# kepingbi/ProdSearch

Measured on AMD Instinct MI355X. Metric: train (u,q,i,neg) tuples/sec at bs=384, 20 neg, d=128, higher is better.
Workload: dtype f32 (fp32 MFMA and VALU; wide products, the fused per-replica kernels and grouped weight gradients as fp32-grade bf16x3 products: exact 3-way bf16 split of both fp32 operands, 6 of the 9 cross products as bf16 MFMAs per step, fp32 accumulation); 1 GPU; item_transformer d=128 1 layer 8 heads ff=512 uprev=20 bs=384/GPU 20 neg Q=8 W=1 P=18357 V=32387 dropout=0.10 (BASELINE configs[1]); global_batch=384, parallelism=dp1, step=sample+fwd+bwd+clip/Adam via nn.Module API (trainer.py:74-78), replicas_per_row=21

## Files before the change

include/prodsearch_hip.h:

```cpp
#ifndef PRODSEARCH_HIP_H
#define PRODSEARCH_HIP_H

#include <stddef.h>
#include <stdint.h>

#ifdef __cplusplus
extern "C" {
#endif

#define PS_MAX_LAYERS 8
#define PS_OK 0
#define PS_ERR_ARG 1
#define PS_ERR_HIP 2

typedef void* ps_stream_t;

enum { PS_MODEL_TEM = 0, PS_MODEL_QEM = 1,
       PS_MODEL_AEM = 2,
       PS_MODEL_ZAM = 3 };
enum { PS_QENC_FS = 0, PS_QENC_AVG = 1 };

typedef struct PsTemDesc {
  int32_t B;
  int32_t K;
// ... 48 lines not shown
  const int64_t *target_prod_idxs;
  const int64_t *u_item_idxs;
  const int64_t *pos_iword_idxs;
  const int64_t *neg_item_idxs;
  const int64_t *neg_word_idxs;
  const int64_t *candi_prod_idxs;
} PsTemBatch;

typedef struct PsTemWsLayout {
  int64_t total_floats;
  int32_t R;
  int32_t S;
  int64_t qmean, query_emb, x;
  int64_t kp, vp, qp, attn, ctx;
  int64_t y1, ln1, a1, h1, y2, enc;
  int64_t item_scores, word_scores, loss_parts;
  int64_t denc, dx;
} PsTemWsLayout;

const char* ps_version(void);
const char* ps_last_error(void);
const char* ps_arith_info(void);
int ps_set_fuse_bwd_min(int rows);
int ps_set_side_mode(int mode);
int ps_side_values_in_use(void);
void ps_side_abort(void);
void ps_debug_fail_fork(int nth);
int ps_set_deterministic(int on);
int ps_gemm_x3_config(int mode, int force_shape);
int ps_gemm_f32_weight(const float* A, int lda, const float* W, int tb, float* C, int ldc, int M, int N, int K,
                       const float* bias, float alpha, ps_stream_t stream);

int ps_tem_workspace_layout(const PsTemDesc* desc, PsTemWsLayout* out);

int ps_tem_forward(const PsTemDesc* desc, const PsTemTensors* params, const PsTemBatch* batch,
                   float* workspace, float* loss3, float* loss_acc, ps_stream_t stream);
int ps_tem_forward_sampled(const PsTemDesc* desc, const PsTemTensors* params, const PsTemBatch* batch,
                           const float* alias_prob, const int32_t* alias_idx, int64_t* neg_item_out, int64_t* neg_word_out,
                           float* workspace, float* loss3, float* loss_acc, ps_stream_t stream);

int ps_tem_backward(const PsTemDesc* desc, const PsTemTensors* params, const PsTemBatch* batch,
                    float* workspace, const PsTemTensors* grads, float loss_scale,
                    const float* loss_scale_dev ,
                    ps_stream_t stream);

int ps_gather_score(const PsTemDesc* desc, const PsTemTensors* params, const PsTemBatch* batch,
// ... 209 lines not shown
```

prodsearch_amd/_lib.py:

```python
import ctypes as C
import os

from . import build as _build

PS_MAX_LAYERS = 8
PS_MODEL_TEM, PS_MODEL_QEM, PS_MODEL_AEM, PS_MODEL_ZAM = 0, 1, 2, 3
PS_QENC_FS, PS_QENC_AVG = 0, 1

_f32p = C.POINTER(C.c_float)
_i64p = C.POINTER(C.c_int64)


class PsTemDesc(C.Structure):
    _fields_ = [(n, C.c_int32) for n in ('B', 'K', 'L', 'Q', 'W', 'C', 'd', 'H', 'F', 'n_layers')] + \
               [('product_size', C.c_int64), ('vocab_size', C.c_int64)] + \
               [(n, C.c_int32) for n in ('model', 'query_encoder', 'use_pos_emb', 'use_item_pos',
                                         'bias_product', 'pos_weight', 'sep_prod_emb', 'training')] + \
               [('dropout', C.c_float), ('seed', C.c_uint64), ('step', C.c_uint64)]


LAYER_FIELDS = ('wk', 'bk', 'wv', 'bv', 'wq', 'bq', 'wo', 'bo', 'w1', 'b1', 'w2', 'b2',
                'ff_ln_g', 'ff_ln_b', 'ln_g', 'ln_b')
TOP_FIELDS = ('product_emb', 'hist_product_emb', 'word_emb', 'product_bias', 'word_bias',
              'fs_w', 'fs_b', 'pe', 'final_ln_g', 'final_ln_b')
# ... 57 lines not shown


class PsRtmTensors(C.Structure):
    _fields_ = [(n, C.c_void_p) for n in RTM_TOP_FIELDS] + [('layer', PsLayerTensors * PS_MAX_LAYERS)]


class PsRtmBatch(C.Structure):
    _fields_ = [(n, C.c_void_p) for n in RTM_BATCH_FIELDS]


class PsRtmWsLayout(C.Structure):
    _fields_ = [('total_floats', C.c_int64)] + [(n, C.c_int32) for n in ('Bseq', 'S', 'J', 'pad_')] + \
               [(n, C.c_int64) for n in ('query_emb', 'valid', 'x', 'vec', 'cnt', 'enc', 'scores', 'weight',
                                         'pv_scores', 'dx')]


PS_RENC_PV, PS_RENC_PVC, PS_RENC_FS, PS_RENC_AVG = 0, 1, 2, 3

SYMBOLS = {
    'ps_version': (C.c_char_p, []),
    'ps_last_error': (C.c_char_p, []),
    'ps_arith_info': (C.c_char_p, []),
    'ps_set_fuse_bwd_min': (C.c_int, [C.c_int]),
    'ps_set_side_mode': (C.c_int, [C.c_int]),
    'ps_side_values_in_use': (C.c_int, []),
    'ps_set_deterministic': (C.c_int, [C.c_int]),
    'ps_side_abort': (None, []),
    'ps_debug_fail_fork': (None, [C.c_int]),
    'ps_gemm_x3_config': (C.c_int, [C.c_int, C.c_int]),
    'ps_gemm_f32_weight': (C.c_int, [C.c_void_p, C.c_int, C.c_void_p, C.c_int, C.c_void_p, C.c_int, C.c_int, C.c_int, C.c_int,
                                     C.c_void_p, C.c_float, C.c_void_p]),
    'ps_tem_workspace_layout': (C.c_int, [C.POINTER(PsTemDesc), C.POINTER(PsTemWsLayout)]),
    'ps_tem_forward': (C.c_int, [C.POINTER(PsTemDesc), C.POINTER(PsTemTensors), C.POINTER(PsTemBatch),
                                 C.c_void_p, C.c_void_p, C.c_void_p, C.c_void_p]),
    'ps_tem_forward_sampled': (C.c_int, [C.POINTER(PsTemDesc), C.POINTER(PsTemTensors), C.POINTER(PsTemBatch),
                                         C.c_void_p, C.c_void_p, C.c_void_p, C.c_void_p, C.c_void_p, C.c_void_p, C.c_void_p,
                                         C.c_void_p]),
    'ps_tem_backward': (C.c_int, [C.POINTER(PsTemDesc), C.POINTER(PsTemTensors), C.POINTER(PsTemBatch),
                                  C.c_void_p, C.POINTER(PsTemTensors), C.c_float, C.c_void_p, C.c_void_p]),
    'ps_gather_score': (C.c_int, [C.POINTER(PsTemDesc), C.POINTER(PsTemTensors), C.POINTER(PsTemBatch),
                                  C.c_void_p, C.c_void_p]),
    'ps_tem_score': (C.c_int, [C.POINTER(PsTemDesc), C.POINTER(PsTemTensors), C.POINTER(PsTemBatch),
                               C.c_void_p, C.c_void_p, C.c_void_p]),
    'ps_rtm_workspace_floats': (C.c_int, [C.POINTER(PsRtmDesc), C.c_int32, C.POINTER(C.c_int64)]),
    'ps_rtm_workspace_layout': (C.c_int, [C.POINTER(PsRtmDesc), C.c_int32, C.POINTER(PsRtmWsLayout)]),
    'ps_rtm_forward': (C.c_int, [C.POINTER(PsRtmDesc), C.POINTER(PsRtmTensors), C.POINTER(PsRtmBatch),
# ... 181 lines not shown
```

prodsearch_amd/csrc/mlp_fused.hip:

```cpp
#include "rowwise.h"
#include "x3frag.h"
#include <stdlib.h>
#ifndef TRY
#define TRY(x) do { int _rc = (x); if (_rc) return _rc; } while (0)
#endif

bool ps_fusion_enabled() {
  static const bool on = ps_env_int("PS_NO_FUSE", 0) == 0;
  return on;
}

#define MD 128
#define MBM 32
#define MT_THREADS 512
#define MLP_PF_DEFAULT 3
#define PLD 132

__device__ inline int opaque(int v) { asm volatile("" : "+v"(v)); return v; }

struct MlpTLds {
  uint16_t Xa[3][MBM * MD];
  float Ps[8][MBM * PLD];
  float vec[6][MD];
  float red[16];
// ... 366 lines not shown
  PS_REQUIRE(mlp_x3_enabled(a.F) && a.M > 0, "fused mlp: F=%d M=%d (F must be 256, 512 or 1024)", a.F, a.M);
  PS_REQUIRE(a.x3.on && a.x3.fwd_wo && a.x3.fwd_ff, "fused mlp: the weight fragment streams are missing (WSplit)");
  PS_REQUIRE(!a.fold_score || mlp_fwd_can_fold_score(a.M, a.F, MD), "fused mlp: folded scoring needs <= 65535 workgroups");
  KTimeScope kt("mlp_fwd", st);
  MlpFwdArgs as = a;
  as.stamp = g_mlp_stamp;
  const dim3 grid(ps_cdiv(a.M, MBM)), block(MT_THREADS);
  static bool a1 = false, a2 = false, a4 = false;
#ifdef PS_DIAG
  static bool ad1 = false, ad2 = false, ad3 = false;
  static const int diag = ps_diag_int("PS_MLP_DIAG", 0);
  if (a.F == 512 && diag == 1) { TRY(set_lds_attr(mlp_fwd_t_kernel<2, 3, 1>, ad1)); PS_KLAUNCH((mlp_fwd_t_kernel<2, 3, 1>), grid, block, sizeof(MlpTLds), st, as); }
  else if (a.F == 512 && diag == 2) { TRY(set_lds_attr(mlp_fwd_t_kernel<2, 3, 2>, ad2)); PS_KLAUNCH((mlp_fwd_t_kernel<2, 3, 2>), grid, block, sizeof(MlpTLds), st, as); }
  else if (a.F == 512 && diag == 3) { TRY(set_lds_attr(mlp_fwd_t_kernel<2, 3, 3>, ad3)); PS_KLAUNCH((mlp_fwd_t_kernel<2, 3, 3>), grid, block, sizeof(MlpTLds), st, as); }
  else
#endif
  if (a.F == 256) { TRY(set_lds_attr(mlp_fwd_t_kernel<1, 3>, a1)); PS_KLAUNCH((mlp_fwd_t_kernel<1, 3>), grid, block, sizeof(MlpTLds), st, as); }
  else if (a.F == 512) { TRY(set_lds_attr(mlp_fwd_t_kernel<2, 3>, a2)); PS_KLAUNCH((mlp_fwd_t_kernel<2, 3>), grid, block, sizeof(MlpTLds), st, as); }
  else { TRY(set_lds_attr(mlp_fwd_t_kernel<4, 3>, a4)); PS_KLAUNCH((mlp_fwd_t_kernel<4, 3>), grid, block, sizeof(MlpTLds), st, as); }
  PS_LAUNCH_CHECK();
  return PS_OK;
}

template <int NBW, int PF>
__global__ __launch_bounds__(MT_THREADS, 2) void mlp_bwd_t_kernel(const MlpBwdArgs a) {
  fork_signal(a.sig, a.sigval);
  extern __shared__ float lds_raw[];
  MlpTLds& L = *reinterpret_cast<MlpTLds*>(lds_raw);
  const int tid = threadIdx.x, lane = tid & 63, wave = __builtin_amdgcn_readfirstlane(tid >> 6), l31 = lane & 31, h = lane >> 5;
  const int m0 = blockIdx.x * MBM, M = a.M, F = a.F;
  const int mrow = 4 * wave + (lane >> 4), c8 = 8 * (lane & 15);
  const int mg = m0 + mrow;
  const bool ok = mg < M;
  const uint32_t step_ctx = drop_step(a.drop_ctx), step_ff1 = drop_step(a.drop_ff1), step_ff2 = drop_step(a.drop_ff2);
  MLP_STAMP(0);
  float (*Csum)[MBM][MD] = reinterpret_cast<float (*)[MBM][MD]>(&L.Ps[2][0]);
  static_assert(3 * MBM * MD <= 3 * MBM * PLD, "column-sum scratch must fit three partial slots");

  const uint16_t* ff_stream = a.x3.bwd_ff + (size_t)(wave * NBW) * 16 * 1536;
  uint4 ring[PF][3];
#pragma unroll
  for (int s = 0; s < PF; ++s) load_frag(ring[s], ff_stream, s, lane);
  if (tid < 64) {
    const int which = tid >> 5, q = tid & 31;
    *reinterpret_cast<float4*>(&L.vec[which][4 * q]) = *reinterpret_cast<const float4*>((which == 0 ? a.gf : a.g1) + 4 * q);
  }
  float x2[8], st2[2] = {0.f, 0.f};
  {
    const float* src = a.y2 + (size_t)(ok ? mg : 0) * MD + c8;
    const float4 v0 = ok ? *reinterpret_cast<const float4*>(src) : make_float4(0.f, 0.f, 0.f, 0.f);
    const float4 v1 = ok ? *reinterpret_cast<const float4*>(src + 4) : make_float4(0.f, 0.f, 0.f, 0.f);
    x2[0] = v0.x; x2[1] = v0.y; x2[2] = v0.z; x2[3] = v0.w; x2[4] = v1.x; x2[5] = v1.y; x2[6] = v1.z; x2[7] = v1.w;
    if (ok) { const float2 s2 = *reinterpret_cast<const float2*>(a.stf + 2 * (size_t)mg); st2[0] = s2.x; st2[1] = s2.y; }
  }
  float dy[8];
  if (a.item_scores) {
    const float invB = a.scale * (a.scale_dev ? *a.scale_dev : 1.f) / (float)a.B;
    const float wpos = a.pos_weight ? (float)a.K : 1.f;
    const int K1 = a.K + 1;
    const int mm = ok ? mg : 0;
    const int b = mm / K1, j = mm - b * K1;
    int64_t idx = j == 0 ? a.target[b] : a.neg_items[(size_t)b * a.K + j - 1];
    idx = idx < 0 ? a.P : (idx > a.P ? a.P : idx);
    const float sc = a.item_scores[mm];
    const float ds = ok ? (j == 0 ? wpos * (sigmoid_f(sc) - 1.f) : sigmoid_f(sc)) * invB : 0.f;
    const float* row = a.product_emb + (size_t)idx * MD + c8;
    const float4 v0 = *reinterpret_cast<const float4*>(row), v1 = *reinterpret_cast<const float4*>(row + 4);
    dy[0] = ds * v0.x; dy[1] = ds * v0.y; dy[2] = ds * v0.z; dy[3] = ds * v0.w;
    dy[4] = ds * v1.x; dy[5] = ds * v1.y; dy[6] = ds * v1.z; dy[7] = ds * v1.w;
  } else {
    const float* src = a.denc + (size_t)(ok ? mg : 0) * MD + c8;
    const float4 v0 = ok ? *reinterpret_cast<const float4*>(src) : make_float4(0.f, 0.f, 0.f, 0.f);
    const float4 v1 = ok ? *reinterpret_cast<const float4*>(src + 4) : make_float4(0.f, 0.f, 0.f, 0.f);
    dy[0] = v0.x; dy[1] = v0.y; dy[2] = v0.z; dy[3] = v0.w; dy[4] = v1.x; dy[5] = v1.y; dy[6] = v1.z; dy[7] = v1.w;
  }
  __syncthreads();
  MLP_STAMP(1);

  auto ln_bwd_stage = [&](const float (&dyv)[8], const float (&x)[8], const float mean, const float rstd, const int vg,
                          const bool has_res, const float (&res)[8], const DropSpec& drop, const uint32_t dstep,
                          float (&dxr)[8], float* out_dx, float* out_drop) {
    const float4 g0 = *reinterpret_cast<const float4*>(&L.vec[vg][c8]), g1 = *reinterpret_cast<const float4*>(&L.vec[vg][c8 + 4]);
    const float gg[8] = {g0.x, g0.y, g0.z, g0.w, g1.x, g1.y, g1.z, g1.w};
    float xh[8], dh[8], s1 = 0.f, s2 = 0.f;
#pragma unroll
    for (int j = 0; j < 8; ++j) {
      xh[j] = (x[j] - mean) * rstd;
      dh[j] = dyv[j] * gg[j];
      s1 += dh[j]; s2 += dh[j] * xh[j];
    }
    s1 = row16_sum(s1) * (1.f / MD);
    s2 = row16_sum(s2) * (1.f / MD);
// ... 54 lines not shown
  park(a.part_f);
  __syncthreads();
  MLP_STAMP(3);

  f32x16 acc2[4];
#pragma unroll
  for (int nb = 0; nb < 4; ++nb)
#pragma unroll
    for (int r = 0; r < 16; ++r) acc2[nb][r] = 0.f;
  const int mrow_p = m0 + l31;
  const bool row_ok = mrow_p < M;
  constexpr int NS = 16 * NBW;
#pragma unroll
  for (int bi = 0; bi < NBW; ++bi) {
    const int fb = wave * NBW + bi, f0 = 32 * fb + 16 * h;
    float* tile = &L.Ps[wave][0];
    float4 a1g[4];
    tile_load(a1g, a.a1 + (size_t)m0 * F + 32 * fb, F, lane, M - m0);
    f32x16 acc1;
#pragma unroll
    for (int r = 0; r < 16; ++r) acc1[r] = 0.f;
    uint4 bq[2][3];
    read_b(bq[0], L.Xa, l31, 8 * h);
    { if ((wave >= 4) == (bi == 0)) __builtin_amdgcn_s_setprio(2); else __builtin_amdgcn_s_setprio(1); }
#pragma unroll
    for (int t = 0; t < 8; ++t) {
      const int s = 16 * bi + t;
      if (t + 1 < 8) read_b(bq[(t + 1) & 1], L.Xa, l31, 16 * (t + 1) + 8 * h);
      __builtin_amdgcn_sched_barrier(0);
      x3_mma(acc1, ring[s % PF], bq[t & 1]);
      load_frag(ring[s % PF], ff_stream, s + PF < NS ? s + PF : NS - 1, lane);
      __builtin_amdgcn_sched_barrier(0);
    }
    { if ((wave >= 4) == (bi == 0)) __builtin_amdgcn_s_setprio(1); else __builtin_amdgcn_s_setprio(0); }
    MLP_STAMP(4 + 2 * bi);
    Philox4 r0 = {0u, 0u, 0u, 0u}, r1 = {0u, 0u, 0u, 0u};
    if (a.drop_ff1.thr) {
      r0 = drop_call16(a.drop_ff1, (uint32_t)mrow_p, (uint32_t)(f0 >> 3), step_ff1);
      r1 = drop_call16(a.drop_ff1, (uint32_t)mrow_p, (uint32_t)(f0 >> 3) + 1u, step_ff1);
    }
    float a1v[16];
    tile_load_put(tile, a1g, lane);
    tile_get(tile, a1v, l31, h);
    float dv[16];
#pragma unroll
    for (int r = 0; r < 16; ++r) {
// ... 1 lines not shown
      if (a.drop_ff1.thr) g *= drop_half(a.drop_ff1, r < 8 ? r0 : r1, r & 7);
      dv[r] = row_ok ? g : 0.f;
    }
    tile_put(tile + MBM * TLD, dv, l31, h);
    tile_store(tile + MBM * TLD, a.da1 + (size_t)m0 * F + 32 * fb, F, lane, M - m0);
    {
      float cs[16];
#pragma unroll
      for (int r = 0; r < 16; ++r) cs[r] = half_sum_last(dv[r]);
      if (l31 == 31) {
        float* pb = a.part_b1 + ((size_t)blockIdx.x * 3) * F + f0;
#pragma unroll
        for (int q = 0; q < 4; ++q) *reinterpret_cast<float4*>(pb + 4 * q) = make_float4(cs[4 * q], cs[4 * q + 1], cs[4 * q + 2], cs[4 * q + 3]);
      }
    }
    MLP_STAMP(5 + 2 * bi);
    { if ((wave >= 4) == (bi == 0)) __builtin_amdgcn_s_setprio(2); else __builtin_amdgcn_s_setprio(1); }
    uint4 df[2][3];
    {
      const float lo8[8] = {dv[0], dv[1], dv[2], dv[3], dv[4], dv[5], dv[6], dv[7]};
      const float hi8[8] = {dv[8], dv[9], dv[10], dv[11], dv[12], dv[13], dv[14], dv[15]};
      split8(lo8, df[0]);
      split8(hi8, df[1]);
    }
#pragma unroll
    for (int u = 0; u < 8; ++u) {
      const int s = 16 * bi + 8 + u;
      x3_mma(acc2[u & 3], ring[s % PF], df[u >> 2]);
      load_frag(ring[s % PF], ff_stream, s + PF < NS ? s + PF : NS - 1, lane);
      __builtin_amdgcn_sched_barrier(0);
    }
  }
  __builtin_amdgcn_s_setprio(0);
  MLP_STAMP(8);
  float x1[8], st1v[2] = {0.f, 0.f};
  {
    const float* src = a.y1 + (size_t)(ok ? mg : 0) * MD + c8;
    const float4 v0 = ok ? *reinterpret_cast<const float4*>(src) : make_float4(0.f, 0.f, 0.f, 0.f);
    const float4 v1 = ok ? *reinterpret_cast<const float4*>(src + 4) : make_float4(0.f, 0.f, 0.f, 0.f);
    x1[0] = v0.x; x1[1] = v0.y; x1[2] = v0.z; x1[3] = v0.w; x1[4] = v1.x; x1[5] = v1.y; x1[6] = v1.z; x1[7] = v1.w;
    if (ok) { const float2 s2 = *reinterpret_cast<const float2*>(a.st1 + 2 * (size_t)mg); st1v[0] = s2.x; st1v[1] = s2.y; }
  }
  const int kbo = wave & 3, nh = wave >> 2;
  const uint16_t* wo_stream = a.x3.bwd_wo + (size_t)(kbo * 8 + 4 * nh) * 1536;
  uint4 wof[4][3];
#pragma unroll
// ... 32 lines not shown
    dump_acc(L.Ps[nh], acc, l31, h, kbo);
  }
  __syncthreads();
  MLP_STAMP(12);
  if (ok) {
    const float* p0 = &L.Ps[0][mrow * PLD + c8];
    const float* p1 = &L.Ps[1][mrow * PLD + c8];
    const float4 u0 = *reinterpret_cast<const float4*>(p0), u1 = *reinterpret_cast<const float4*>(p0 + 4);
    const float4 w0 = *reinterpret_cast<const float4*>(p1), w1 = *reinterpret_cast<const float4*>(p1 + 4);
    float* q = a.dctx + (size_t)mg * MD + c8;
    *reinterpret_cast<float4*>(q) = make_float4(u0.x + w0.x, u0.y + w0.y, u0.z + w0.z, u0.w + w0.w);
    *reinterpret_cast<float4*>(q + 4) = make_float4(u1.x + w1.x, u1.y + w1.y, u1.z + w1.z, u1.w + w1.w);
  }
  MLP_STAMP(13);
}

int mlp_bwd_fused_blocks(int M) { return ps_cdiv(M, MBM); }
int mlp_bwd_b1_rows(int M, int F) { (void)F; return ps_cdiv(M, MBM); }

int launch_mlp_bwd_fused(const MlpBwdArgs& a, hipStream_t st) {
  PS_REQUIRE(mlp_x3_enabled(a.F) && a.M > 0, "fused mlp backward: F=%d M=%d (F must be 256, 512 or 1024)", a.F, a.M);
  PS_REQUIRE(a.part_f && a.part_1 && a.part_b1, "fused mlp backward: column sums must be parked");
  PS_REQUIRE(a.x3.on && a.x3.bwd_wo && a.x3.bwd_ff, "fused mlp backward: the weight fragment streams are missing (WSplit)");
  KTimeScope kt("mlp_bwd", st);
  MlpBwdArgs b = a;
  b.sig = nullptr; b.sigval = 0;
  b.stamp = g_mlp_stamp ? g_mlp_stamp + 128 : nullptr;
  const dim3 grid(ps_cdiv(a.M, MBM)), block(MT_THREADS);
  static bool a1 = false, a2 = false, a4 = false;
  if (a.F == 256) TRY(set_lds_attr(mlp_bwd_t_kernel<1, 3>, a1));
  else if (a.F == 512) TRY(set_lds_attr(mlp_bwd_t_kernel<2, 3>, a2));
  else TRY(set_lds_attr(mlp_bwd_t_kernel<4, 3>, a4));
  side_take_signal(st, &b.sig, &b.sigval);
  if (a.F == 256) hipLaunchKernelGGL((mlp_bwd_t_kernel<1, 3>), grid, block, sizeof(MlpTLds), st, b);
  else if (a.F == 512) hipLaunchKernelGGL((mlp_bwd_t_kernel<2, 3>), grid, block, sizeof(MlpTLds), st, b);
  else hipLaunchKernelGGL((mlp_bwd_t_kernel<4, 3>), grid, block, sizeof(MlpTLds), st, b);
  PS_LAUNCH_CHECK();
  return PS_OK;
}
```

prodsearch_amd/csrc/rowwise.h:

```cpp
#pragma once
#include "common.h"

struct ScoreArgs {
  int B, K, W, C, R, d;
  FDiv fK1, fWK1, fC;
  int64_t P, V;
  int bias_product, pos_weight;
  const int64_t* target; const int64_t* neg_items; const int64_t* pos_words; const int64_t* neg_words;
  const int64_t* candi;
  const float* product_emb; const float* word_emb; const float* product_bias; const float* word_bias;
  const float* enc;
  float* item_scores;
  float* word_scores;
  float* loss_parts;
  float* item_terms;
  float* word_terms;
  float* loss3;
  float* loss_acc;
  float* loss_blk;
  int loss_nblk;
  float scale;
  const float* scale_dev;
  float* denc;
  int part;
  float* g_product_emb; float* g_word_emb; float* g_product_bias; float* g_word_bias;
  float* word_blk; int word_nblk; float* item_blk; uint32_t* ticket;
  const float* samp_prob; const int32_t* samp_alias; uint32_t samp_step, samp_k0, samp_k1; int samp_inline;
  unsigned long long* stamp;
};
#define PS_WORD_TASKS_PER_WG 16
inline void score_finish(ScoreArgs& a) {
  a.fK1 = make_fdiv(a.K + 1); a.fWK1 = make_fdiv(a.W * (a.K + 1)); a.fC = make_fdiv(a.C > 0 ? a.C : 1);
}
int launch_score_fwd(ScoreArgs& a, hipStream_t st);
int launch_loss(const ScoreArgs& a, hipStream_t st);
int launch_score_bwd(const ScoreArgs& a, hipStream_t st);

struct WSplit {
  const float* w[3]; int rows[3], cols[3];
  uint16_t* fwd_wo; uint16_t* fwd_ff; uint16_t* bwd_ff; uint16_t* bwd_wo;
  int on;
  const float* wkv[2]; uint16_t* fwd_kv;
  uint16_t* bwd_kv;
};
__host__ __device__ inline int wsplit_chunks(const WSplit& W, int ) {
  const int d = W.cols[0], F = W.rows[1];
  return (d * d + 2 * d * F) / 8 + (W.wkv[0] ? 2 * d * d / 8 : 0);
// ... 205 lines not shown
struct MlpFwdArgs {
  int M, F;
  int fan, S, qpos;
  const float* ctx; const float* xin;
  const float *wo, *bo, *g1, *be1, *w1, *b1, *w2, *b2, *gf, *bef;
  DropSpec drop_ctx, drop_ff1, drop_ff2;
  float *y1, *ln1, *st1, *a1, *h1, *y2, *stf, *enc;
  int fold_score; ScoreArgs sc;
  WSplit x3;
  unsigned long long* stamp;
};
int launch_mlp_fwd_fused(const MlpFwdArgs& a, hipStream_t st);
bool mlp_fwd_can_fold_score(int M, int F, int d);
bool mlp_x3_enabled(int F);
bool mlp_fused_serves(int d, int F);
int64_t mlp_x3_floats(int d, int F);
bool ps_fusion_enabled();

struct MlpBwdArgs {
  int M, F;
  const float* denc;
  const float* item_scores; const int64_t* target; const int64_t* neg_items; const float* product_emb;
  int B, K, pos_weight; int64_t P; float scale; const float* scale_dev;
  const float* y2; const float* stf; const float* gf;
  const float* y1; const float* st1; const float* g1;
  const float* a1;
  const float *wo, *w1, *w2;
  DropSpec drop_ctx, drop_ff1, drop_ff2;
  float* do2;
  float* da1;
  float* dy1;
  float* dout;
  float* dctx;
  float* part_f;
  float* part_1;
  float* part_b1;
  WSplit x3;
  uint32_t* sig; uint32_t sigval;
  unsigned long long* stamp;
};
int launch_mlp_bwd_fused(const MlpBwdArgs& a, hipStream_t st);
int mlp_bwd_fused_blocks(int M);
int mlp_bwd_b1_rows(int M, int F);
```

prodsearch_amd/csrc/rowwise.hip:

```cpp
#include "rowwise.h"
#include <stdlib.h>

static inline int lpr_for(int d) {
  int n = d / 4, l = 1;
  while (l < n && l < 64) l <<= 1;
  return l;
}

__device__ inline int64_t clamp_idx(int64_t i, int64_t hi) { return i < 0 ? hi : (i > hi ? hi : i); }

struct Task {
  const float* row; const float* vec; float bias; float* out;
  float* term; float tw;
  float lw;
};
__device__ inline Task score_task(const ScoreArgs& a, int t) {
  Task k;
  const int K1 = a.K + 1;
  if (a.C > 0) {
    int b = fdiv(t, a.fC);
    int64_t idx = clamp_idx(a.candi[t], a.P);
    k.row = a.product_emb + (size_t)idx * a.d;
    k.vec = a.enc + (size_t)b * a.R * a.d;
    k.bias = a.bias_product ? a.product_bias[idx] : 0.f;
// ... 1438 lines not shown
      it.bias = 0.f;
    });
  det_owner_walk<EPL, WG>(a.B * a.W * K1, owner, nown, hl, d, a.g_word_emb, a.g_word_bias, a.V - 1, keys_word,
    [&](int u, DetItem& it) {
      const int b = fdiv(u, a.fWK1), r = u - b * a.W * K1, w = r / K1, j = r - w * K1;
      it.row = keys_word[u];
      const float s = a.word_scores[((size_t)b * a.W + w) * K1 + j];
      const float* prow = a.product_emb + (size_t)clamp_idx(a.target[b], a.P) * d;
      float pv[EPL];
#pragma unroll
      for (int k = 0; k < EPL; ++k) pv[k] = (WG && k < epl) ? prow[c + 32 * k] : 0.f;
      int cnt = 0;
      for (int w2 = 0; w2 < a.W; ++w2) cnt += (a.pos_words[(size_t)b * a.W + w2] != a.V - 1);
      const float ds = (j == 0 ? sigmoid_f(s) - 1.f : sigmoid_f(s)) * (invB / (float)(cnt > 0 ? cnt : 1));
#pragma unroll
      for (int k = 0; k < EPL; ++k) it.v[k] = ds * pv[k];
      it.bias = ds;
    });
}

int launch_score_bwd(const ScoreArgs& a, hipStream_t st) {
  PS_REQUIRE(a.d % 32 == 0 && a.d <= 32 * BW_MAXE, "score bwd: d=%d unsupported", a.d);
  if (ps_deterministic()) {
    if (a.denc && a.part != 2) {
      ScoreArgs e = a;
      e.part = 1;
      const int iw = a.R > 1 ? ps_cdiv(a.B * (a.K + 1), SB_RG) : 0;
      launch_score_bwd_kernel(e, (a.R > 1 ? 2 : 1) * a.B + iw, st);
      PS_LAUNCH_CHECK();
    }
    if (a.part != 1) {
      const size_t nkeys = (size_t)a.B * (a.K + 1) * (1 + a.W) + a.B;
      float* term = ps_det_scratch(1, (size_t)a.B * a.d + nkeys + 4, st);
      PS_REQUIRE(term, "score bwd: deterministic mode has no scratch (allocation failed or stream capture)");
      int32_t* keys = reinterpret_cast<int32_t*>(term + (size_t)a.B * a.d);
      hipLaunchKernelGGL(score_bwd_det_pre_kernel, dim3(ps_cdiv(a.B, 8)), dim3(256), 0, st, a, term, keys);
      PS_LAUNCH_CHECK();
      if (a.g_word_emb) {
        if (a.d <= 128) hipLaunchKernelGGL(score_bwd_det_kernel<4>, dim3(256), dim3(32 * SBD_OWNERS_PER_WG), 0, st, a, term, keys);
        else if (a.d <= 256) hipLaunchKernelGGL(score_bwd_det_kernel<8>, dim3(256), dim3(32 * SBD_OWNERS_PER_WG), 0, st, a, term, keys);
        else hipLaunchKernelGGL(score_bwd_det_kernel<16>, dim3(256), dim3(32 * SBD_OWNERS_PER_WG), 0, st, a, term, keys);
      } else {
        if (a.d <= 128) hipLaunchKernelGGL((score_bwd_det_kernel<4, false>), dim3(256), dim3(32 * SBD_OWNERS_PER_WG), 0, st, a, term, keys);
        else if (a.d <= 256) hipLaunchKernelGGL((score_bwd_det_kernel<8, false>), dim3(256), dim3(32 * SBD_OWNERS_PER_WG), 0, st, a, term, keys);
        else hipLaunchKernelGGL((score_bwd_det_kernel<16, false>), dim3(256), dim3(32 * SBD_OWNERS_PER_WG), 0, st, a, term, keys);
      }
      PS_LAUNCH_CHECK();
    }
    return PS_OK;
  }
  const int item_wgs = a.R > 1 ? ps_cdiv(a.B * (a.K + 1), SB_RG) : 0;
#if PS_DIAG_ON
  ScoreArgs as = a;
  as.stamp = ps_diag_int("PS_SBW_STAMP", 0) ? ps_debug_stamp_ptr() : nullptr;
  launch_score_bwd_kernel(as, (a.R > 1 ? 2 : 1) * a.B + item_wgs, st);
#else
  launch_score_bwd_kernel(a, (a.R > 1 ? 2 : 1) * a.B + item_wgs, st);
#endif
  PS_LAUNCH_CHECK();
  return PS_OK;
}

template <int EPL>
__device__ __forceinline__ void row_fetch_add(float* dst, const float* src, int c, float scale) {
  float v[EPL];
#pragma unroll
  for (int k = 0; k < EPL; ++k) v[k] = src[c + 32 * k];
#pragma unroll
  for (int k = 0; k < EPL; ++k) atomicAdd(&dst[c + 32 * k], scale == 1.f ? v[k] : v[k] * scale);
}
template <int EPL>
__device__ __forceinline__ void row_fetch_add2(float* dst, const float* src, const float* src2, int c) {
  float v[EPL], u[EPL];
#pragma unroll
// ... 455 lines not shown
```

prodsearch_amd/csrc/tem.hip:

```cpp
#include "encoder.h"
#include "graph.h"
#include <math.h>
#include <stdarg.h>
#include <stdio.h>
#include <string.h>

static thread_local char g_err[512] = "";
void ps_set_error(const char* fmt, ...) {
  va_list ap;
  va_start(ap, fmt);
  vsnprintf(g_err, sizeof(g_err), fmt, ap);
  va_end(ap);
}
extern "C" const char* ps_last_error(void) { return g_err; }
extern "C" const char* ps_version(void) { return "prodsearch_hip 0.1 (gfx950, fp32 MFMA)"; }
bool gemm_x3_on();
extern "C" const char* ps_arith_info(void) {
  return gemm_x3_on() ? "f32 (fp32 MFMA and VALU; wide products, the fused per-replica kernels and grouped weight gradients as fp32-grade "
                        "bf16x3 products: exact 3-way bf16 split of both fp32 operands, 6 of the 9 cross products as bf16 MFMAs per step, "
                        "fp32 accumulation)"
                      : "f32 (fp32 MFMA and VALU)";
}

#include <vector>
// ... 969 lines not shown
  PS_CHECK_HIP(hipMemcpyAsync(enc_out, workspace + w.enc, sizeof(float) * (size_t)D.B * D.d, hipMemcpyDeviceToDevice, st));
  return PS_OK;
}

static void park_colsums(LnBwdArgs& a, float* ws, const Ws& w, ColFoldList* fold) {
  if (!fold || fold->n >= PS_MAX_COLFOLD) return;
  ColFold& f = fold->e[fold->n];
  a.partial = ws + w.lnpart + (size_t)fold->n * w.lnrows * 3 * a.d;
  f.partial = a.partial; f.nblk = ln_bwd_blocks(a.rows); f.d = a.d;
  f.dst[0] = a.dgamma; f.dst[1] = a.dbeta; f.dst[2] = a.colsum;
  ++fold->n;
}

static int& fuse_bwd_min_slot() {
  static int v = ps_env_int("PS_FUSE_BWD_MIN", 1024);
  return v;
}
extern "C" int ps_set_fuse_bwd_min(int rows) {
  const int old = fuse_bwd_min_slot();
  fuse_bwd_min_slot() = rows;
  return old;
}

static thread_local GemmProblem g_wg3_last[4];
static thread_local int g_wg3_last_n = 0;
static thread_local bool g_wg3_defer_ok = false;
static int flush_wg3_last(hipStream_t st) {
  const int n = g_wg3_last_n;
  g_wg3_last_n = 0;
  return n ? run_wgrads(g_wg3_last, n, st) : PS_OK;
}
int enc_layers_backward(const PsTemDesc& D, const PsTemTensors& P, const PsTemTensors& G, const int64_t* ui,
                        const float* valid, float* ws, const Ws& w, hipStream_t st, ColFoldList* fold,
                        const ScoreArgs* score_on_side, bool rows_listed) {
  const bool drop = D.training && D.dropout > 0.f;
  const int B = D.B, d = D.d, S = w.S, NL = D.n_layers, F = D.F;
  PS_REQUIRE(G.final_ln_g && G.final_ln_b, "backward: null final LayerNorm gradient");
  LnBwdArgs f;
  memset(&f, 0, sizeof(f));
  f.dy = ws + w.denc; f.lddy = d; f.stats = ws + w.fin_stats; f.g = P.final_ln_g; f.d = d;
  f.dgamma = G.final_ln_g; f.dbeta = G.final_ln_b;
  side_set_light((int64_t)B * S * d <= ((int64_t)2 << 20));
  static const bool bwd_fuse_on = ps_env_int("PS_NO_FUSE_BWD", 0) == 0;
  const int bwd_fuse_min = fuse_bwd_min_slot();
  const bool fuse_last = NL > 0 && fold && bwd_fuse_on && ps_fusion_enabled() && w.layer[NL - 1].Sq == 1 &&
                         mlp_fused_serves(d, F) && w.wsplit && w.layer[NL - 1].M2 == w.Mf && w.Mf >= bwd_fuse_min &&
                         mlp_bwd_fused_blocks(w.Mf) <= w.lnrows && fold->n + 3 <= PS_MAX_COLFOLD;
  if (score_on_side && !(fuse_last && w.R > 1)) {
    ScoreArgs t = *score_on_side;
    t.denc = ws + w.denc;
    SideCtx* sc = side_ctx_on(st);
    if (sc && w.R > 1) {
      t.part = 1;
      TRY(launch_score_bwd(t, st));
      TRY(side_fork(st));
      t.part = 2;
      TRY(launch_score_bwd(t, sc->stream));
    } else {
      TRY(launch_score_bwd(t, st));
    }
    score_on_side = nullptr;
  }
  if (fuse_last) {
  } else if (NL > 0) {
    const LayerWs& l = w.layer[NL - 1];
    f.x = ws + l.y2; f.ldx = d; f.rows = w.Mf; f.dx = ws + w.dy2; f.lddx = d;
    f.colsum = G.layer[NL - 1].b2;
// ... 12 lines not shown
    const PsLayerTensors& Lp = P.layer[i];
    const PsLayerTensors& Lg = G.layer[i];
    PS_REQUIRE(Lg.wk && Lg.wv && Lg.wq && Lg.wo && Lg.w1 && Lg.w2 && Lg.bk && Lg.bv && Lg.bq && Lg.bo && Lg.b1 &&
               Lg.b2 && Lg.ff_ln_g && Lg.ff_ln_b, "backward: layer %d has null gradients", i);
    const float* xin = i == 0 ? ws + w.x : ws + w.layer[i - 1].y2;
    const float* xn = ws + l.xn;
    const int ns = l.n_in * S, M2 = l.M2;
    const float* do2 = drop ? ws + w.do2 : ws + w.dy2;
    const bool fused = fuse_last && i == NL - 1;
    static const bool wgrad_early = ps_diag_int("PS_WGRAD_LATE", 0) == 0;
    if (fused) {
      MlpBwdArgs m;
      memset(&m, 0, sizeof(m));
      m.M = M2; m.F = F;
      m.denc = ws + w.denc; m.y2 = ws + l.y2; m.stf = ws + w.fin_stats; m.gf = P.final_ln_g;
      m.y1 = ws + l.y1; m.st1 = ws + l.ff_stats; m.g1 = Lp.ff_ln_g; m.a1 = ws + l.a1;
      m.wo = Lp.wo; m.w1 = Lp.w1; m.w2 = Lp.w2;
      m.drop_ctx = make_drop(D, PS_SITE_CTX(i)); m.drop_ff1 = make_drop(D, PS_SITE_FF1(i));
      m.drop_ff2 = make_drop(D, PS_SITE_FF2(i));
      if (score_on_side) {
        const ScoreArgs& sa = *score_on_side;
        m.item_scores = sa.item_scores; m.target = sa.target; m.neg_items = sa.neg_items; m.product_emb = sa.product_emb;
        m.B = sa.B; m.K = sa.K; m.pos_weight = sa.pos_weight; m.P = sa.P; m.scale = sa.scale; m.scale_dev = sa.scale_dev;
      }
      m.x3 = make_wsplit(D, P, ws, w);
      m.do2 = const_cast<float*>(do2); m.da1 = ws + w.da1; m.dy1 = ws + w.dy1;
      m.dout = drop ? ws + w.do_ : ws + w.dy1; m.dctx = ws + w.dctx;
      const int nwg = mlp_bwd_fused_blocks(M2);
      {
        ColFold& c0 = fold->e[fold->n];
        m.part_f = ws + w.lnpart + (size_t)fold->n * w.lnrows * 3 * d;
        c0.partial = m.part_f; c0.nblk = nwg; c0.d = d;
        c0.dst[0] = G.final_ln_g; c0.dst[1] = G.final_ln_b; c0.dst[2] = Lg.b2;
        ++fold->n;
        ColFold& c1 = fold->e[fold->n];
        m.part_1 = ws + w.lnpart + (size_t)fold->n * w.lnrows * 3 * d;
        c1.partial = m.part_1; c1.nblk = nwg; c1.d = d;
        c1.dst[0] = Lg.ff_ln_g; c1.dst[1] = Lg.ff_ln_b; c1.dst[2] = Lg.bo;
        ++fold->n;
        ColFold& c2 = fold->e[fold->n];
        m.part_b1 = ws + w.gcpart;
        c2.partial = m.part_b1; c2.nblk = mlp_bwd_b1_rows(M2, F); c2.d = F;
        c2.dst[0] = Lg.b1; c2.dst[1] = nullptr; c2.dst[2] = nullptr;
        ++fold->n;
      }
      TRY(launch_mlp_bwd_fused(m, st));
      GemmProblem wg[1] = {gp_wgrad(do2, d, ws + l.h1, F, Lg.w2, d, F, M2)};
      GemmProblem wg1[1] = {gp_wgrad(ws + w.da1, F, ws + l.ln1, d, Lg.w1, F, d, M2)};
      GemmProblem wgo[1] = {gp_wgrad(m.dout, d, ws + l.ctx, d, Lg.wo, d, d, M2)};
      TRY(side_fork(st));
      if (score_on_side) {
        ScoreArgs t = *score_on_side;
        t.denc = nullptr;
        SideCtx* sc = side_ctx_on(st);
        TRY(launch_score_bwd(t, sc ? sc->stream : st));
      }
      static const int wg_group_rows = ps_diag_int("PS_WGRAD_GROUP_ROWS", (1 << 30));
      if (M2 <= wg_group_rows) {
        GemmProblem all3[3] = {wg[0], wg1[0], wgo[0]};
        TRY(side_run(all3, 3, st));
      } else {
        TRY(side_run(wg, 1, st));
        TRY(side_run(wg1, 1, st));
        TRY(side_run(wgo, 1, st));
      }
    } else {
      GemmProblem p = gp(do2, d, 0, Lp.w2, F, 1, ws + w.da1, F, M2, F, d);
      p.act = ACT_GELU_BWD; p.act_aux = ws + l.a1; p.drop = make_drop(D, PS_SITE_FF1(i)); p.colsum = Lg.b1;
      if (fold && fold->n < PS_MAX_COLFOLD && i == NL - 1) {
        ColFold& cf = fold->e[fold->n++];
        p.colsum_part = ws + w.gcpart;
        cf.partial = p.colsum_part; cf.nblk = 4 * ps_cdiv(M2, 64); cf.d = F;
        cf.dst[0] = Lg.b1; cf.dst[1] = nullptr; cf.dst[2] = nullptr;
      }
// ... 143 lines not shown
      if (drop) { n.out2 = ws + w.do2; n.drop2 = make_drop(D, PS_SITE_FF2(i - 1)); }
      n.colsum = G.layer[i - 1].b2; n.dgamma = Lg.ln_g; n.dbeta = Lg.ln_b;
      park_colsums(n, ws, w, fold);
      TRY(launch_ln_bwd(n, st));
    }
  }
  return PS_OK;
}

static int tem_backward_impl(const PsTemDesc* desc, const PsTemTensors* params, const PsTemBatch* batch,
                             float* ws, const PsTemTensors* grads, float loss_scale, const float* loss_scale_dev,
                             ps_stream_t stream);
extern "C" int ps_tem_backward(const PsTemDesc* desc, const PsTemTensors* params, const PsTemBatch* batch,
                               float* ws, const PsTemTensors* grads, float loss_scale, const float* loss_scale_dev,
                               ps_stream_t stream) {
  const int rc = tem_backward_impl(desc, params, batch, ws, grads, loss_scale, loss_scale_dev, stream);
  if (rc != PS_OK) { side_abort(); enc_clear_call_flags(); }
  return rc;
}
static int tem_backward_impl(const PsTemDesc* desc, const PsTemTensors* params, const PsTemBatch* batch,
                             float* ws, const PsTemTensors* grads, float loss_scale, const float* loss_scale_dev,
                             ps_stream_t stream) {
  enc_clear_call_flags();
  PS_REQUIRE(desc && params && batch && ws && grads, "backward: null argument");
  PsTemDesc D = *desc;
  D.C = 0;
  Ws w;
  TRY(make_ws(D, w));
  hipStream_t st = (hipStream_t)stream;
  const PsTemTensors& P = *params;
  const PsTemTensors& G = *grads;
  const bool tem = D.model == PS_MODEL_TEM;
  const bool drop = D.training && D.dropout > 0.f;
  const int B = D.B, d = D.d, S = w.S, NL = tem ? D.n_layers : 0, F = D.F;
  const float* hist = D.sep_prod_emb ? P.hist_product_emb : P.product_emb;
  float* ghist = D.sep_prod_emb ? G.hist_product_emb : G.product_emb;
  const bool word_grad = G.word_emb != nullptr;
  PS_REQUIRE(G.product_emb && G.word_bias && ghist && hist, "backward: null table gradient");
  PS_REQUIRE(!D.bias_product || G.product_bias, "backward: null product_bias gradient");

  ScoreArgs s;
  fill_score(D, P, *batch, ws, w, s);
  s.scale = loss_scale; s.scale_dev = loss_scale_dev; s.denc = ws + w.denc;
  s.g_product_emb = G.product_emb; s.g_word_emb = G.word_emb; s.g_product_bias = G.product_bias;
  s.g_word_bias = G.word_bias;
  static const bool score_side_on = ps_diag_int("PS_SCORE_BWD_MAIN", 0) == 0;
  const bool score_deferred = tem && NL > 0 && w.R > 1 && score_side_on;
  if (!score_deferred) TRY(launch_score_bwd(s, st));

  const float* wp_w[PS_WPLANES_MAX]; int wp_r[PS_WPLANES_MAX], wp_c[PS_WPLANES_MAX];
  const int wp_n = wplane_list(D, P, w, wp_w, wp_r, wp_c);
  WPlaneScope wplanes(st, wp_w, wp_r, wp_c, wp_n);
  ColFoldList fold;
  fold.n = 0;
  const float* dqe = ws + w.denc;
  int lddqe = d;
  if (tem) {
    g_wg3_defer_ok = true; g_wg3_last_n = 0;
    const int rc_enc = enc_layers_backward(D, P, G, batch->u_item_idxs, nullptr, ws, w, st, &fold, score_deferred ? &s : nullptr,
                                           rows_list_ok(D));
    g_wg3_defer_ok = false;
    if (rc_enc != PS_OK) { g_wg3_last_n = 0; return rc_enc; }
    dqe = ws + w.dx;
    lddqe = S * d;
  } else if (ps_model_attn(D.model)) {
    TRY(ae_backward(D, P, G, batch->u_item_idxs, ws, w, st));
    dqe = ws + w.ae_dqe;
  }

  bool fw_by_gemm = false;
  EmbedBwdArgs e;
  memset(&e, 0, sizeof(e));
  e.B = B; e.Q = D.Q; e.L = D.L; e.S = S; e.d = d; e.P = D.product_size; e.V = D.vocab_size; e.tem = tem;
  e.qw = batch->query_word_idxs; e.ui = batch->u_item_idxs; e.dx = ws + w.dx;
  if (enc_take_dx_two_partials()) e.dx2 = ws + w.dxn;
  e.drop_fs = make_drop(D, PS_SITE_FS);
  e.g_hist_tab = ghist; e.g_word_emb = G.word_emb;
  if (D.query_encoder == PS_QENC_FS) {
    PS_REQUIRE(G.fs_w && G.fs_b, "backward: null FS encoder gradient");
    e.fw_x = ws + w.qmean; e.g_fs_w = G.fs_w;
    if (ps_fusion_enabled() && d <= 128) {
      e.fsb_dqe = dqe; e.fsb_lddqe = lddqe; e.fsb_qe = ws + w.query_emb; e.fsb_w = P.fs_w; e.g_fs_b = G.fs_b;
      if (word_grad) e.det_dm = ws + w.dqmean;
      static const bool fw_gemm_on = ps_env_int("PS_FW_BY_GEMM", 1) != 0;
// ... 1 lines not shown
    } else {
      TRY(launch_tanh_bwd(dqe, lddqe, ws + w.query_emb, ws + w.dqpre, G.fs_b, B, d, st));
      if (word_grad) {
        GemmProblem p = gp(ws + w.dqpre, d, 0, P.fs_w, d, 1, ws + w.dqmean, d, B, d, d);
        p.no_deep = 1;
        TRY(run1(p, st));
        e.dqmean_d = ws + w.dqmean;
      }
      e.fw_dy = ws + w.dqpre;
    }
  } else if (word_grad) {
    PS_CHECK_HIP(hipMemcpy2DAsync(ws + w.dqmean, sizeof(float) * d, dqe, sizeof(float) * lddqe, sizeof(float) * d, B,
                                  hipMemcpyDeviceToDevice, st));
    e.dqmean_d = ws + w.dqmean;
  }
  e.fold = fold;
  const int rc_sc = launch_embed_scatter(e, st);
  if (rc_sc != PS_OK) { g_wg3_last_n = 0; return rc_sc; }
  if (fw_by_gemm) {
    PS_REQUIRE(g_wg3_last_n <= 3, "backward: deferred weight-gradient group is full");
    g_wg3_last[g_wg3_last_n++] = gp_wgrad(ws + w.dqpre, d, ws + w.qmean, d, G.fs_w, d, d, B);
  }
  TRY(flush_wg3_last(st));
  TRY(side_join(st));
  return PS_OK;
}

struct StageLayout { uint32_t* step_word; int64_t* p[6]; int n[6]; };
static StageLayout stage_layout(const PsTemDesc& D, float* ws, const Ws& w) {
  StageLayout L;
  L.step_word = reinterpret_cast<uint32_t*>(ws + w.stage);
  int64_t* base = reinterpret_cast<int64_t*>(ws + w.stage + 4);
  const int n[6] = {D.B * D.Q, D.B * D.L, D.B, D.B * D.W, D.B * D.K, D.B * D.W * D.K};
  int64_t off = 0;
  for (int k = 0; k < 6; ++k) { L.p[k] = base + off; L.n[k] = n[k]; off += (n[k] + 1) & ~1; }
  return L;
}
static PsTemBatch staged_batch(const StageLayout& L) {
  PsTemBatch b;
  memset(&b, 0, sizeof(b));
  b.query_word_idxs = L.p[0]; b.u_item_idxs = L.p[1]; b.target_prod_idxs = L.p[2]; b.pos_iword_idxs = L.p[3];
  b.neg_item_idxs = L.p[4]; b.neg_word_idxs = L.p[5];
  return b;
}

extern "C" int ps_graph_replay_enabled(void) { return ps_graphs_enabled() ? 1 : 0; }
// ... 182 lines not shown
```

Before: 35.22 million tuples/s.

## Fuse item-embedding gradient scatter into the fused MLP backward kernel

Adds a templated ISC path to the fused MLP backward kernel. Each wave reads the score gradient and item index per row and atomically adds ds*enc into the product-embedding and bias gradients, interleaved with the MFMA loop. The separate score backward on the side stream then skips the item rows and only handles word gradients, launched after the deferred weight-gradient flush. This removes a separate item-scatter pass and its reread of enc. In exchange it adds atomics and registers inside a hot kernel and moves the word scatter later, onto the main stream.

```diff
diff --git a/include/prodsearch_hip.h b/include/prodsearch_hip.h
--- a/include/prodsearch_hip.h
+++ b/include/prodsearch_hip.h
@@ -94,6 +94,8 @@
 const char* ps_last_error(void);
 const char* ps_arith_info(void);
 int ps_set_fuse_bwd_min(int rows);
+int ps_set_item_scatter_fused(int on);
+int ps_item_scatter_fused_taken(void);
 int ps_set_side_mode(int mode);
 int ps_side_values_in_use(void);
 void ps_side_abort(void);
diff --git a/prodsearch_amd/_lib.py b/prodsearch_amd/_lib.py
--- a/prodsearch_amd/_lib.py
+++ b/prodsearch_amd/_lib.py
@@ -103,6 +103,8 @@
     'ps_last_error': (C.c_char_p, []),
     'ps_arith_info': (C.c_char_p, []),
     'ps_set_fuse_bwd_min': (C.c_int, [C.c_int]),
+    'ps_set_item_scatter_fused': (C.c_int, [C.c_int]),
+    'ps_item_scatter_fused_taken': (C.c_int, []),
     'ps_set_side_mode': (C.c_int, [C.c_int]),
     'ps_side_values_in_use': (C.c_int, []),
     'ps_set_deterministic': (C.c_int, [C.c_int]),
diff --git a/prodsearch_amd/csrc/mlp_fused.hip b/prodsearch_amd/csrc/mlp_fused.hip
--- a/prodsearch_amd/csrc/mlp_fused.hip
+++ b/prodsearch_amd/csrc/mlp_fused.hip
@@ -412,7 +412,7 @@
   return PS_OK;
 }
 
-template <int NBW, int PF>
+template <int NBW, int PF, bool ISC>
 __global__ __launch_bounds__(MT_THREADS, 2) void mlp_bwd_t_kernel(const MlpBwdArgs a) {
   fork_signal(a.sig, a.sigval);
   extern __shared__ float lds_raw[];
@@ -435,6 +435,21 @@
     const int which = tid >> 5, q = tid & 31;
     *reinterpret_cast<float4*>(&L.vec[which][4 * q]) = *reinterpret_cast<const float4*>((which == 0 ? a.gf : a.g1) + 4 * q);
   }
+  float isc_e[4][2], isc_ds[4]; int isc_idx[4]; bool isc_live[4];
+  if (ISC) {
+#pragma unroll
+    for (int r = 0; r < 4; ++r) {
+      const int mr = m0 + 4 * wave + r;
+      const float* er = a.enc + (size_t)(mr < M ? mr : 0) * MD + lane;
+      isc_e[r][0] = er[0]; isc_e[r][1] = er[64];
+    }
+  }
+  auto isc_add = [&](const int r) {
+    float* g = a.g_product_emb + (size_t)isc_idx[r] * MD + lane;
+    atomicAdd(g, isc_live[r] ? isc_ds[r] * isc_e[r][0] : 0.f);
+    atomicAdd(g + 64, isc_live[r] ? isc_ds[r] * isc_e[r][1] : 0.f);
+    if (a.g_product_bias && lane == 0) atomicAdd(&a.g_product_bias[isc_idx[r]], isc_ds[r]);
+  };
   float x2[8], st2[2] = {0.f, 0.f};
   {
     const float* src = a.y2 + (size_t)(ok ? mg : 0) * MD + c8;
@@ -458,6 +473,14 @@
     const float4 v0 = *reinterpret_cast<const float4*>(row), v1 = *reinterpret_cast<const float4*>(row + 4);
     dy[0] = ds * v0.x; dy[1] = ds * v0.y; dy[2] = ds * v0.z; dy[3] = ds * v0.w;
     dy[4] = ds * v1.x; dy[5] = ds * v1.y; dy[6] = ds * v1.z; dy[7] = ds * v1.w;
+    if (ISC) {
+#pragma unroll
+      for (int r = 0; r < 4; ++r) {
+        isc_ds[r] = __builtin_bit_cast(float, __builtin_amdgcn_readlane(__builtin_bit_cast(int, ds), 16 * r));
+        isc_idx[r] = __builtin_amdgcn_readlane((int)idx, 16 * r);
+        isc_live[r] = m0 + 4 * wave + r < M && isc_idx[r] != (int)a.P;
+      }
+    }
   } else {
     const float* src = a.denc + (size_t)(ok ? mg : 0) * MD + c8;
     const float4 v0 = ok ? *reinterpret_cast<const float4*>(src) : make_float4(0.f, 0.f, 0.f, 0.f);
@@ -558,6 +581,10 @@
     for (int r = 0; r < 16; ++r) acc1[r] = 0.f;
     uint4 bq[2][3];
     read_b(bq[0], L.Xa, l31, 8 * h);
+    if (ISC) {
+#pragma unroll
+      for (int r = 0; r < 4; ++r) if (r * NBW / 2 == 2 * bi) isc_add(r);
+    }
     { if ((wave >= 4) == (bi == 0)) __builtin_amdgcn_s_setprio(2); else __builtin_amdgcn_s_setprio(1); }
 #pragma unroll
     for (int t = 0; t < 8; ++t) {
@@ -605,6 +632,10 @@
       const float hi8[8] = {dv[8], dv[9], dv[10], dv[11], dv[12], dv[13], dv[14], dv[15]};
       split8(lo8, df[0]);
       split8(hi8, df[1]);
+    }
+    if (ISC) {
+#pragma unroll
+      for (int r = 0; r < 4; ++r) if (r * NBW / 2 == 2 * bi + 1) isc_add(r);
     }
 #pragma unroll
     for (int u = 0; u < 8; ++u) {
@@ -683,19 +714,33 @@
   PS_REQUIRE(mlp_x3_enabled(a.F) && a.M > 0, "fused mlp backward: F=%d M=%d (F must be 256, 512 or 1024)", a.F, a.M);
   PS_REQUIRE(a.part_f && a.part_1 && a.part_b1, "fused mlp backward: column sums must be parked");
   PS_REQUIRE(a.x3.on && a.x3.bwd_wo && a.x3.bwd_ff, "fused mlp backward: the weight fragment streams are missing (WSplit)");
+  const bool isc = a.g_product_emb != nullptr;
+  PS_REQUIRE(!isc || (a.item_scores && a.enc && a.M == a.B * (a.K + 1)), "fused mlp backward: the item scatter needs the scores, enc and M = B (K + 1)");
   KTimeScope kt("mlp_bwd", st);
   MlpBwdArgs b = a;
   b.sig = nullptr; b.sigval = 0;
   b.stamp = g_mlp_stamp ? g_mlp_stamp + 128 : nullptr;
   const dim3 grid(ps_cdiv(a.M, MBM)), block(MT_THREADS);
-  static bool a1 = false, a2 = false, a4 = false;
-  if (a.F == 256) TRY(set_lds_attr(mlp_bwd_t_kernel<1, 3>, a1));
-  else if (a.F == 512) TRY(set_lds_attr(mlp_bwd_t_kernel<2, 3>, a2));
-  else TRY(set_lds_attr(mlp_bwd_t_kernel<4, 3>, a4));
+  static bool a1 = false, a2 = false, a4 = false, s1 = false, s2 = false, s4 = false;
+  if (isc) {
+    if (a.F == 256) TRY(set_lds_attr(mlp_bwd_t_kernel<1, 3, true>, s1));
+    else if (a.F == 512) TRY(set_lds_attr(mlp_bwd_t_kernel<2, 3, true>, s2));
+    else TRY(set_lds_attr(mlp_bwd_t_kernel<4, 3, true>, s4));
+  } else {
+    if (a.F == 256) TRY(set_lds_attr(mlp_bwd_t_kernel<1, 3, false>, a1));
+    else if (a.F == 512) TRY(set_lds_attr(mlp_bwd_t_kernel<2, 3, false>, a2));
+    else TRY(set_lds_attr(mlp_bwd_t_kernel<4, 3, false>, a4));
+  }
   side_take_signal(st, &b.sig, &b.sigval);
-  if (a.F == 256) hipLaunchKernelGGL((mlp_bwd_t_kernel<1, 3>), grid, block, sizeof(MlpTLds), st, b);
-  else if (a.F == 512) hipLaunchKernelGGL((mlp_bwd_t_kernel<2, 3>), grid, block, sizeof(MlpTLds), st, b);
-  else hipLaunchKernelGGL((mlp_bwd_t_kernel<4, 3>), grid, block, sizeof(MlpTLds), st, b);
+  if (isc) {
+    if (a.F == 256) hipLaunchKernelGGL((mlp_bwd_t_kernel<1, 3, true>), grid, block, sizeof(MlpTLds), st, b);
+    else if (a.F == 512) hipLaunchKernelGGL((mlp_bwd_t_kernel<2, 3, true>), grid, block, sizeof(MlpTLds), st, b);
+    else hipLaunchKernelGGL((mlp_bwd_t_kernel<4, 3, true>), grid, block, sizeof(MlpTLds), st, b);
+  } else {
+    if (a.F == 256) hipLaunchKernelGGL((mlp_bwd_t_kernel<1, 3, false>), grid, block, sizeof(MlpTLds), st, b);
+    else if (a.F == 512) hipLaunchKernelGGL((mlp_bwd_t_kernel<2, 3, false>), grid, block, sizeof(MlpTLds), st, b);
+    else hipLaunchKernelGGL((mlp_bwd_t_kernel<4, 3, false>), grid, block, sizeof(MlpTLds), st, b);
+  }
   PS_LAUNCH_CHECK();
   return PS_OK;
 }
diff --git a/prodsearch_amd/csrc/rowwise.h b/prodsearch_amd/csrc/rowwise.h
--- a/prodsearch_amd/csrc/rowwise.h
+++ b/prodsearch_amd/csrc/rowwise.h
@@ -23,6 +23,7 @@
   const float* scale_dev;
   float* denc;
   int part;
+  int items_elsewhere;
   float* g_product_emb; float* g_word_emb; float* g_product_bias; float* g_word_bias;
   float* word_blk; int word_nblk; float* item_blk; uint32_t* ticket;
   const float* samp_prob; const int32_t* samp_alias; uint32_t samp_step, samp_k0, samp_k1; int samp_inline;
@@ -274,6 +275,7 @@
   const float* denc;
   const float* item_scores; const int64_t* target; const int64_t* neg_items; const float* product_emb;
   int B, K, pos_weight; int64_t P; float scale; const float* scale_dev;
+  const float* enc; float* g_product_emb; float* g_product_bias;
   const float* y2; const float* stf; const float* gf;
   const float* y1; const float* st1; const float* g1;
   const float* a1;
diff --git a/prodsearch_amd/csrc/rowwise.hip b/prodsearch_amd/csrc/rowwise.hip
--- a/prodsearch_amd/csrc/rowwise.hip
+++ b/prodsearch_amd/csrc/rowwise.hip
@@ -1484,6 +1484,7 @@
 int launch_score_bwd(const ScoreArgs& a, hipStream_t st) {
   PS_REQUIRE(a.d % 32 == 0 && a.d <= 32 * BW_MAXE, "score bwd: d=%d unsupported", a.d);
   if (ps_deterministic()) {
+    PS_REQUIRE(!a.items_elsewhere, "score bwd: the deterministic scatter owns the item rows too");
     if (a.denc && a.part != 2) {
       ScoreArgs e = a;
       e.part = 1;
@@ -1511,7 +1512,8 @@
     }
     return PS_OK;
   }
-  const int item_wgs = a.R > 1 ? ps_cdiv(a.B * (a.K + 1), SB_RG) : 0;
+  PS_REQUIRE(!a.items_elsewhere || (a.R > 1 && a.part == 0 && !a.denc), "score bwd: items_elsewhere needs replicas, part 0 and no d enc");
+  const int item_wgs = a.R > 1 && !a.items_elsewhere ? ps_cdiv(a.B * (a.K + 1), SB_RG) : 0;
 #if PS_DIAG_ON
   ScoreArgs as = a;
   as.stamp = ps_diag_int("PS_SBW_STAMP", 0) ? ps_debug_stamp_ptr() : nullptr;
diff --git a/prodsearch_amd/csrc/tem.hip b/prodsearch_amd/csrc/tem.hip
--- a/prodsearch_amd/csrc/tem.hip
+++ b/prodsearch_amd/csrc/tem.hip
@@ -1015,9 +1015,22 @@
   return old;
 }
 
+static int& item_scatter_fused_slot() {
+  static int v = ps_env_int("PS_ITEM_SCATTER_FUSED", 1);
+  return v;
+}
+extern "C" int ps_set_item_scatter_fused(int on) {
+  const int old = item_scatter_fused_slot();
+  item_scatter_fused_slot() = on;
+  return old;
+}
+static int g_item_scatter_taken = 0;
+extern "C" int ps_item_scatter_fused_taken(void) { return g_item_scatter_taken; }
+
 static thread_local GemmProblem g_wg3_last[4];
 static thread_local int g_wg3_last_n = 0;
 static thread_local bool g_wg3_defer_ok = false;
+static thread_local bool g_score_words_last = false;
 static int flush_wg3_last(hipStream_t st) {
   const int n = g_wg3_last_n;
   g_wg3_last_n = 0;
@@ -1036,6 +1049,7 @@
   side_set_light((int64_t)B * S * d <= ((int64_t)2 << 20));
   static const bool bwd_fuse_on = ps_env_int("PS_NO_FUSE_BWD", 0) == 0;
   const int bwd_fuse_min = fuse_bwd_min_slot();
+  g_item_scatter_taken = 0;
   const bool fuse_last = NL > 0 && fold && bwd_fuse_on && ps_fusion_enabled() && w.layer[NL - 1].Sq == 1 &&
                          mlp_fused_serves(d, F) && w.wsplit && w.layer[NL - 1].M2 == w.Mf && w.Mf >= bwd_fuse_min &&
                          mlp_bwd_fused_blocks(w.Mf) <= w.lnrows && fold->n + 3 <= PS_MAX_COLFOLD;
@@ -1094,6 +1108,10 @@
         const ScoreArgs& sa = *score_on_side;
         m.item_scores = sa.item_scores; m.target = sa.target; m.neg_items = sa.neg_items; m.product_emb = sa.product_emb;
         m.B = sa.B; m.K = sa.K; m.pos_weight = sa.pos_weight; m.P = sa.P; m.scale = sa.scale; m.scale_dev = sa.scale_dev;
+        if (item_scatter_fused_slot() != 0 && !ps_deterministic() && g_wg3_defer_ok && sa.part == 0 && sa.enc && sa.g_product_emb) {
+          m.enc = sa.enc; m.g_product_emb = sa.g_product_emb;
+          m.g_product_bias = sa.bias_product ? sa.g_product_bias : nullptr;
+        }
       }
       m.x3 = make_wsplit(D, P, ws, w);
       m.do2 = const_cast<float*>(do2); m.da1 = ws + w.da1; m.dy1 = ws + w.dy1;
@@ -1121,7 +1139,10 @@
       GemmProblem wg1[1] = {gp_wgrad(ws + w.da1, F, ws + l.ln1, d, Lg.w1, F, d, M2)};
       GemmProblem wgo[1] = {gp_wgrad(m.dout, d, ws + l.ctx, d, Lg.wo, d, d, M2)};
       TRY(side_fork(st));
-      if (score_on_side) {
+      if (score_on_side && m.g_product_emb) {
+        g_score_words_last = true;
+        g_item_scatter_taken = 1;
+      } else if (score_on_side) {
         ScoreArgs t = *score_on_side;
         t.denc = nullptr;
         SideCtx* sc = side_ctx_on(st);
@@ -1311,6 +1332,7 @@
                              float* ws, const PsTemTensors* grads, float loss_scale, const float* loss_scale_dev,
                              ps_stream_t stream) {
   enc_clear_call_flags();
+  g_item_scatter_taken = 0;
   PS_REQUIRE(desc && params && batch && ws && grads, "backward: null argument");
   PsTemDesc D = *desc;
   D.C = 0;
@@ -1342,13 +1364,16 @@
   WPlaneScope wplanes(st, wp_w, wp_r, wp_c, wp_n);
   ColFoldList fold;
   fold.n = 0;
+  bool score_words_last = false;
   const float* dqe = ws + w.denc;
   int lddqe = d;
   if (tem) {
-    g_wg3_defer_ok = true; g_wg3_last_n = 0;
+    g_wg3_defer_ok = true; g_wg3_last_n = 0; g_score_words_last = false;
     const int rc_enc = enc_layers_backward(D, P, G, batch->u_item_idxs, nullptr, ws, w, st, &fold, score_deferred ? &s : nullptr,
                                            rows_list_ok(D));
     g_wg3_defer_ok = false;
+    score_words_last = g_score_words_last;
+    g_score_words_last = false;
     if (rc_enc != PS_OK) { g_wg3_last_n = 0; return rc_enc; }
     dqe = ws + w.dx;
     lddqe = S * d;
@@ -1396,6 +1421,11 @@
     g_wg3_last[g_wg3_last_n++] = gp_wgrad(ws + w.dqpre, d, ws + w.qmean, d, G.fs_w, d, d, B);
   }
   TRY(flush_wg3_last(st));
+  if (score_words_last) {
+    ScoreArgs t = s;
+    t.denc = nullptr; t.items_elsewhere = 1;
+    TRY(launch_score_bwd(t, st));
+  }
   TRY(side_join(st));
   return PS_OK;
 }
```

Result: faster. 36.66 million tuples/s (median of 6 runs) (+4.1%).
